# matthewygf/GPUSchedule

Hardware: NVIDIA H100
Metric: simulated events/sec (100k-job trace, 4x32x8 cluster) (higher is better)
Workload: dtype int32/int64 (+f64 durations)

## Files before the change

### gpuschedule_b200/csrc/gs_common.cuh

```cuda
#pragma once

#ifndef GS_TICK_MINBLOCKS
#define GS_TICK_MINBLOCKS 28
#endif
#ifndef GS_POLICY_MINBLOCKS
#define GS_POLICY_MINBLOCKS 20
#endif
#define FULL 0xffffffffu


struct __align__(32) JobIn {
  int arrive;
  int gpus;
  int gpc;
  int ps;
  long long memb;
  double dur;
};

struct PJob {
  int last_check, total_exec, exec, pending, last_pending, start, resume;
  unsigned char status, q_id, pad0, pad1;
};
enum { PST_NONE = 0, PST_PENDING = 1, PST_RUNNING = 2, PST_END = 3 };

struct SimDev {
  int M, G, K;
  int netcost, n, wheel_mask, policy, pad0;
  long long cap_bytes;
  long long fit_limit;
  double bandwidth, latency;
  const JobIn *jobs;
  const double *model_mb, *iters;
  gs_job_rec *rec;
  int *jstart;
  double *dur2;
  struct JobState2 *jst2;
  int *stack, *fin, *wheel_head;
  long long *wheel_mem;
  void *spans;
  gs_tick_row *rows;
  gs_evrow *evrows;
  gs_qrow *qrows;
  gs_nodeev *nodeev;
  unsigned long long *nbusy;
  int *nk;
  long long span_cap, rows_cap, qrows_cap;
  struct PJob *pj;
  int *runnable, *queues, *endj, *tmpl, *cidle, *ckfree;
  int *stalej;
  const double *git_data, *git_index;
  const double *git_direct;
  long long git_direct_n;
  double queue_limit[GS_MAX_QUEUES];
  double gittins_delta, next_gittins_unit;
  int num_queue, git_n, rn, en, end_time, next_job_jump, stale_n, qn[GS_MAX_QUEUES];
  int comm_rank, comm_n;
  int comm_min_runnable, comm_pad;
  long long comm_cap;
  double *comm_rk_in;
  unsigned long long *comm_flags;
  double *comm_peer_rk[GS_MAX_RANKS];
  unsigned long long *comm_peer_flags[GS_MAX_RANKS];
  unsigned long long comm_epoch;
  long long comm_wait_cycles;
  int delta, p, top, running, finished, ever, busy_gpus, done, status, need_init;
  int blocked;
  int nev, nq;
  int nne;
  long long mem_busy, sum_arr, span_used, events, evals, started, ticks, row_first;
};

#define EVER_BIT 0x80000000u
```

### gpuschedule_b200/csrc/gs_tick2.cuh

```cuda
#pragma once

#define SCACHE 4

struct __align__(16) JobState2 {
  int next;
  int where;
  unsigned long long mask0;
};

__device__ __forceinline__ unsigned lds32(unsigned a) { unsigned v; asm volatile("ld.shared.u32 %0, [%1];" : "=r"(v) : "r"(a)); return v; }
__device__ __forceinline__ void sts32(unsigned a, unsigned v) { asm volatile("st.shared.u32 [%0], %1;" :: "r"(a), "r"(v)); }
__device__ __forceinline__ unsigned long long lds64(unsigned a) { unsigned long long v; asm volatile("ld.shared.u64 %0, [%1];" : "=l"(v) : "r"(a)); return v; }
__device__ __forceinline__ void sts64(unsigned a, unsigned long long v) { asm volatile("st.shared.u64 [%0], %1;" :: "r"(a), "l"(v)); }
__device__ __forceinline__ int2 ldsv2(unsigned a) { int2 v; asm volatile("ld.shared.v2.s32 {%0, %1}, [%2];" : "=r"(v.x), "=r"(v.y) : "r"(a)); return v; }
__device__ __forceinline__ void stsv2(unsigned a, int2 v) { asm volatile("st.shared.v2.s32 [%0], {%1, %2};" :: "r"(a), "r"(v.x), "r"(v.y)); }

template <bool G64> struct MaskOps;
template <> struct MaskOps<true> {
  typedef unsigned long long T;
  typedef gs_span Span;
  static __device__ __forceinline__ Span make_span(int node, int ntasks, bool first, T mask) {
    Span sp; sp.node = node; sp.ntasks = ntasks | (first ? (int)0x80000000 : 0); sp.devmask = mask; return sp;
  }
  static __device__ __forceinline__ void st_span(Span *p, const Span &v) { __stcs(reinterpret_cast<int4 *>(p), *reinterpret_cast<const int4 *>(&v)); }
  static __device__ __forceinline__ int span_node(const Span &v) { return v.node; }
  static __device__ __forceinline__ int span_ntasks(const Span &v) { return v.ntasks & 0x7fffffff; }
  static __device__ __forceinline__ T span_mask(const Span &v) { return v.devmask; }
  static __device__ __forceinline__ T ld(unsigned a) { return lds64(a); }
  static __device__ __forceinline__ void st(unsigned a, T v) { sts64(a, v); }
  static __device__ __forceinline__ int popc(T v) { return __popcll(v); }
};
template <> struct MaskOps<false> {
  typedef unsigned T;
  typedef gs_cspan Span;
  static __device__ __forceinline__ Span make_span(int node, int ntasks, bool first, T mask) {
    Span sp; sp.where = (unsigned)node | ((unsigned)(ntasks - 1) << 20) | (first ? 0x80000000u : 0u); sp.devmask = mask; return sp;
  }
  static __device__ __forceinline__ void st_span(Span *p, const Span &v) { __stcs(reinterpret_cast<int2 *>(p), *reinterpret_cast<const int2 *>(&v)); }
  static __device__ __forceinline__ int span_node(const Span &v) { return (int)(v.where & 0xfffffu); }
  static __device__ __forceinline__ int span_ntasks(const Span &v) { return (int)((v.where >> 20) & 0x3fu) + 1; }
  static __device__ __forceinline__ T span_mask(const Span &v) { return v.devmask; }
// ... 14 lines not shown
}

__device__ __forceinline__ int meta_cap(unsigned mt, int gpc) {
  const int idle = (int)(mt & 0xffu), kfree = (int)(mt >> 16);
  return min(gpc == 1 ? idle : idle / gpc, kfree);
}

__device__ __forceinline__ int need_of(double dur) {
  const double cl = ceil(dur);
  return cl < 1.0 ? 1 : (cl > 1.0e9 ? 0x7fffffff : (int)cl);
}

#define GS_INF 0x7fffffff

template <bool NET, bool G64>
__global__ void __launch_bounds__(32, GS_TICK_MINBLOCKS) gs_tick2_kernel(SimDev *sims, int nsims, long long max_ticks, int smem_stride) {
  extern __shared__ __align__(16) unsigned char smem_raw[];
  typedef MaskOps<G64> MO;
  typedef typename MO::T MaskT;
  unsigned lane_u;
  asm volatile("mov.u32 %0, %%laneid;" : "=r"(lane_u));
  const int lane = (int)lane_u;
  const int sim = blockIdx.x;
  if (sim >= nsims) return;
  SimDev &S = sims[sim];
  if (S.done || S.status != 0 || S.policy != GS_SCHED_FIFO || (S.netcost != 0) != NET || (S.G > 32) != G64) return;

  const int M = S.M, G = S.G, n = S.n;
  unsigned sb_busy = (unsigned)__cvta_generic_to_shared(smem_raw);
  asm volatile("" : "+r"(sb_busy));
  unsigned sb_kk = sb_busy + 8u * (unsigned)M;
  asm volatile("" : "+r"(sb_kk));
  const unsigned sb_stk = sb_kk + 4u * (unsigned)(M + (M & 1));
#define BUSY_A(nd_) (sb_busy + 8u * (unsigned)(nd_))
#define KK_A(nd_) (sb_kk + 4u * (unsigned)(nd_))
#define STK_A(i_) (sb_stk + 8u * (unsigned)((i_) & (SCACHE - 1)))

  const JobIn *__restrict__ jobs = S.jobs;
  int *jstart = S.jstart;
  JobState2 *jst = S.jst2;
  int2 *stack = reinterpret_cast<int2 *>(S.stack);
  int *fin = S.fin, *whead = S.wheel_head;
  long long *wmem = S.wheel_mem;
  typedef typename MO::Span SpanT;
  SpanT *spans = reinterpret_cast<SpanT *>(S.spans);
  int2 *rowA = reinterpret_cast<int2 *>(S.evrows), *rowB = reinterpret_cast<int2 *>(S.qrows);
  int2 *nodeev = reinterpret_cast<int2 *>(S.nodeev);
  __builtin_assume(__isGlobal(jobs)); __builtin_assume(__isGlobal(jstart)); __builtin_assume(__isGlobal(jst));
  __builtin_assume(__isGlobal(stack)); __builtin_assume(__isGlobal(fin)); __builtin_assume(__isGlobal(whead));
  __builtin_assume(__isGlobal(wmem)); __builtin_assume(__isGlobal(spans)); __builtin_assume(__isGlobal(rowA));
  __builtin_assume(__isGlobal(rowB)); __builtin_assume(__isGlobal(nodeev));
  const int wmask = S.wheel_mask;
  const long long cap_bytes = S.cap_bytes, fit_limit = S.fit_limit;
  const int span_cap = (int)(S.span_cap > 0x7fffffffLL ? 0x7fffffffLL : S.span_cap);
  MaskT gmask = (G >= (int)(8 * sizeof(MaskT))) ? ~(MaskT)0 : (((MaskT)1 << G) - (MaskT)1);
  if constexpr (G64) asm volatile("" : "+l"(gmask));
  else asm volatile("" : "+r"(gmask));

  int delta = S.delta, p = S.p, top = S.top, running = S.running, finished = S.finished;
  int ever = S.ever, busy_gpus = S.busy_gpus, status = 0, blocked = S.blocked;
  int span_used = (int)S.span_used;
  long long mem_busy = S.mem_busy, sum_arr = S.sum_arr, evals = S.evals;
  const int delta0 = delta;
  const int capA = (int)(S.rows_cap > 0x7fffffffLL ? 0x7fffffffLL : S.rows_cap);
  const int capB = (int)(S.qrows_cap > 0x7fffffffLL ? 0x7fffffffLL : S.qrows_cap);
  int na = 0, nb = 0, nne = 0;
  int ever_rec = -1;
  long long budget_ll = max_ticks > 0 ? max_ticks : 0x7fffffffLL;
  if (budget_ll > 0x7fffffffLL - delta - 2) budget_ll = 0x7fffffffLL - delta - 2;
  const int t_end = delta + (int)(budget_ll > 0 ? budget_ll : 0);

  if (S.need_init) {
    const int K = S.K;
    for (int i = lane; i < M; i += 32) { sts64(BUSY_A(i), 0ull); sts32(KK_A(i), (unsigned)G | ((unsigned)K << 16)); }
    for (int i = lane; i <= wmask; i += 32) { whead[i] = -1; wmem[i] = 0; }
  } else {
    const int K = S.K;
    for (int i = lane; i < M; i += 32) {
      const unsigned long long bz = S.nbusy[i];
      const unsigned kv = (unsigned)S.nk[i];
      sts64(BUSY_A(i), bz);
      sts32(KK_A(i), (unsigned)(G - __popcll(bz)) | ((kv & EVER_BIT) ? 0x100u : 0u) | ((unsigned)(K - (int)(kv & ~EVER_BIT)) << 16));
    }
  }
  int scount = top;
  for (int i = max(scount - SCACHE, 0) + lane; i < scount; i += 32) stsv2(STK_A(i), stack[i]);
  int cache_lo = max(scount - SCACHE, 0);
  int bottom_arr = (top > 0) ? stack[0].y : 0;
  __syncwarp();

  int wbase = p & ~31;
  int warr = GS_INF, wpk = 1 | (1 << 24), wneed = 1, wps = 0;
  long long wmemc = 0;
  double wdur = 0.0;
#define LOAD_WINDOW()                                                                         \
  do {                                                                                        \
    warr = GS_INF;                                                                            \
    if (wbase + lane < n) {                                                                   \
      JobIn r_;                                                                               \
      {                                                                                       \
        const int4 *src_ = reinterpret_cast<const int4 *>(&jobs[wbase + lane]);               \
        const int4 v0_ = __ldcs(src_), v1_ = __ldcs(src_ + 1);             \
        r_.arrive = v0_.x; r_.gpus = v0_.y; r_.gpc = v0_.z; r_.ps = v0_.w;                     \
        r_.memb = (long long)(((unsigned long long)(unsigned)v1_.y << 32) | (unsigned)v1_.x); \
        r_.dur = __hiloint2double(v1_.w, v1_.z);                                              \
      }                                                                                       \
      warr = r_.arrive; wpk = r_.gpus | (r_.gpc << 24);                                       \
      wneed = need_of(r_.dur); if (!(r_.memb < fit_limit)) wneed = -wneed;                    \
      wmemc = (long long)r_.gpus * (r_.memb < cap_bytes ? r_.memb : cap_bytes);               \
      if (NET) { wdur = r_.dur; wps = r_.ps; }                                                \
    }                                                                                         \
  } while (0)
  LOAD_WINDOW();
  int next_arr = GS_INF;
  if (p < n) next_arr = __shfl_sync(FULL, warr, p - wbase);

  bool hvalid = false;
  int hjob = -1, harr = 0, hpk = 1 | (1 << 24), hneed = 1, hps = 0;
  long long hmemc = 0;
  double hdur = 0.0;
#define HEAD_FROM_WINDOW(src_)                                                                \
  do {                                                                                        \
    hpk = __shfl_sync(FULL, wpk, (src_)); hneed = __shfl_sync(FULL, wneed, (src_));           \
    hmemc = __shfl_sync(FULL, wmemc, (src_));                                                 \
    if (NET) { hdur = __longlong_as_double(__shfl_sync(FULL, __double_as_longlong(wdur), (src_))); hps = __shfl_sync(FULL, wps, (src_)); } \
  } while (0)

  int next_fin = GS_INF, nf_head = -1;
  JobState2 nf_js; nf_js.next = -1; nf_js.where = 0; nf_js.mask0 = 0ull;
  if (running > 0) {
    int base = delta + 1;
    while (true) {
      const int ph = whead[(base + lane) & wmask];
      const unsigned b = __ballot_sync(FULL, ph >= 0);
      if (b) { const int pos = __ffs(b) - 1; next_fin = base + pos; nf_head = __shfl_sync(FULL, ph, pos); break; }
      base += 32;
    }
    nf_js = jst[nf_head];
  }

  bool done = (n == 0);
  bool force = true;

  while (!done && status == 0) {
    if (na >= capA || nb >= capB) break;
    if (!force && (top == 0 || blocked)) {
      const int t_next = min(next_arr, next_fin - 1);
      if (t_next > delta) {
        const int t_to = min(t_next, t_end);
        if (blocked) evals += (long long)(t_to - delta) * M;
        delta = t_to;
      }
    }
    if (delta >= t_end) break;
    bool changed = force;
    force = false;
    if (next_arr <= delta) {
      int cnt = 0, q = p;
      while (true) {
        const int idx = wbase + lane;
        const unsigned b = __ballot_sync(FULL, idx >= q && warr <= delta);
        const int c = __popc(b);
        if (c > 0 && cnt == 0) {
          if (hvalid) {
            const int2 e = make_int2(hjob, harr);
            stack[scount] = e; stsv2(STK_A(scount), e);
            scount += 1;
          }
          HEAD_FROM_WINDOW(p - wbase);
        }
        cnt += c; q += c;
// ... 12 lines not shown
        if (scount - cache_lo > SCACHE) cache_lo = scount - SCACHE;
        if (top == 0) bottom_arr = delta;
        hjob = p; harr = delta; hvalid = true;
        top += cnt; p += cnt;
        sum_arr += (long long)cnt * delta;
        blocked = 0; changed = true;
        __syncwarp();
      }
      next_arr = GS_INF;
      if (p < n) next_arr = __shfl_sync(FULL, warr, p - wbase);
    }
    if (top > 0 && blocked) evals += M;
    if (top > 0 && !blocked) {
      if (!hvalid) {
        int2 e;
        if (scount - 1 >= cache_lo) e = ldsv2(STK_A(scount - 1));
        else e = stack[scount - 1];
        scount -= 1;
        if (cache_lo > scount) cache_lo = scount;
        hjob = e.x; harr = e.y; hvalid = true;
        if (hjob >= wbase && hjob < wbase + 32) {
          HEAD_FROM_WINDOW(hjob - wbase);
        } else {
          const JobIn jr = jobs[hjob];
          hpk = jr.gpus | (jr.gpc << 24);
          hneed = need_of(jr.dur); if (!(jr.memb < fit_limit)) hneed = -hneed;
          hmemc = (long long)jr.gpus * (jr.memb < cap_bytes ? jr.memb : cap_bytes);
          if (NET) { hdur = jr.dur; hps = jr.ps; }
        }
      }
      const int hg = hpk & 0xffffff, hgpc = (int)((unsigned)hpk >> 24);
      const int htasks = hgpc == 1 ? hg : hg / hgpc;
      const bool placeable = hneed > 0;
      int pre_bk = 0, pre_head = -1;
      long long pre_wm = 0;
      if (!NET && placeable) {
        pre_bk = (delta + min(hneed, wmask)) & wmask;
        pre_head = whead[pre_bk];
        pre_wm = wmem[pre_bk];
      }
      bool ok = false;
      int nspans = 0, where = 0;
      const int span_first = span_used;
      unsigned long long mask0 = 0;
      if (hg <= G) {
        int found = -1;
        for (int base = 0; base < M; base += 32) {
          const int nd = base + lane;
          bool fit = false;
          if (nd < M) {
            const unsigned mt = lds32(KK_A(nd));
            fit = (int)(mt & 0xffu) >= hg && (int)(mt >> 16) >= htasks;
          }
          if (!placeable) {
            if (fit) sts32(KK_A(nd), lds32(KK_A(nd)) - ((unsigned)htasks << 16));
            continue;
          }
          const unsigned b = __ballot_sync(FULL, fit);
          if (b) { found = base + __ffs(b) - 1; break; }
        }
        if (found >= 0 && span_used + 1 > span_cap) { status = GS_ERR_CAPACITY; found = -1; }
        if (found >= 0) {
          ok = true; nspans = 1;
          const MaskT bz = MO::ld(BUSY_A(found));
          const MaskT take = take_lowest<MaskT>(~bz & gmask, hg);
          const unsigned kv = lds32(KK_A(found));
          MO::st(BUSY_A(found), bz | take);
          sts32(KK_A(found), (kv - (unsigned)hg - ((unsigned)htasks << 16)) | 0x100u);
          MO::st_span(&spans[span_first], MO::make_span(found, htasks, true, take));
          mask0 = take;
          where = found | ((htasks - 1) << 20);
          ever += (kv & 0x100u) ? 0 : 1;
          evals += found + 1;
        } else {
          evals += M;
        }
      } else {
// ... 11 lines not shown
            if (nd < M) { const unsigned mt = lds32(KK_A(nd)); if (meta_cap(mt, hgpc) > 0) sts32(KK_A(nd), mt - (1u << 16)); }
          }
        }
        if (last_base >= 0 && (long long)span_used + min(htasks, M) > (long long)span_cap) { status = GS_ERR_CAPACITY; last_base = -1; }
        if (last_base >= 0) {
          ok = true;
          int rem = htasks, last_node = 0;
          for (int base = 0; base <= last_base; base += 32) {
            const int nd = base + lane;
            const unsigned kv = (nd < M) ? lds32(KK_A(nd)) : 0u;
            const int c = meta_cap(kv, hgpc);
            int incl = c;
            #pragma unroll
            for (int o = 1; o < 32; o <<= 1) { const int v = __shfl_up_sync(FULL, incl, o); if (lane >= o) incl += v; }
            const int take = min(c, max(rem - (incl - c), 0));
            const unsigned tb = __ballot_sync(FULL, take > 0);
            bool fresh = false;
            if (take > 0) {
              const MaskT bz = MO::ld(BUSY_A(nd));
              const MaskT tk = take_lowest<MaskT>(~bz & gmask, take * hgpc);
              MO::st(BUSY_A(nd), bz | tk);
              sts32(KK_A(nd), (kv - (unsigned)(take * hgpc) - ((unsigned)take << 16)) | 0x100u);
              fresh = !(kv & 0x100u);
              const int slot = nspans + __popc(tb & ((1u << lane) - 1u));
              MO::st_span(&spans[span_first + slot], MO::make_span(nd, take, slot == 0, tk));
            }
            ever += __popc(__ballot_sync(FULL, fresh));
            if (tb) last_node = base + 31 - __clz(tb);
            nspans += __popc(tb);
            const int tot = __shfl_sync(FULL, incl, 31);
            rem -= min(rem, tot);
          }
          where = (int)0x80000000 | span_first;
          mask0 = (unsigned long long)(unsigned)nspans | ((unsigned long long)(unsigned)hg << 32);
          evals += last_node + 1;
          __syncwarp();
        } else {
          evals += M;
          __syncwarp();
        }
      }
      if (ok) {
        const int j = hjob;
        int need = hneed;
        if (NET) {
          double dur2 = hdur;
          if (hps > 1) {
            const double mps = __ddiv_rn(S.model_mb[j], S.bandwidth);
            const double nis = __dmul_rn((double)nspans, S.latency);
            const double rt = __dmul_rn(S.iters[j], 2.0);
            dur2 = __dadd_rn(hdur, __dmul_rn(__dadd_rn(mps, nis), rt));
          }
          const double eff = dur2 > hdur ? dur2 : hdur;
          need = need_of(eff);
          S.dur2[j] = dur2;
        }
        if (need > wmask) { status = GS_ERR_ARG; need = wmask; }
        const int endt = delta + need;
        const int bk = endt & wmask;
        span_used += nspans;
        JobState2 js; js.where = where; js.mask0 = mask0; js.next = -1;
        if (endt < next_fin) { next_fin = endt; nf_head = j; nf_js = js; }
        else if (endt == next_fin) { js.next = nf_head; nf_head = j; nf_js = js; }
        else js.next = NET ? whead[bk] : pre_head;
        const long long wm = NET ? wmem[bk] : pre_wm;
        whead[bk] = j;
        wmem[bk] = wm + hmemc;
        *reinterpret_cast<int4 *>(&jst[j]) = *reinterpret_cast<const int4 *>(&js);
        __stcs(&jstart[j], delta);
        top -= 1;
        sum_arr -= harr;
        running += 1;
        busy_gpus += hg;
        mem_busy += hmemc;
        hvalid = false; changed = true;
      } else if (placeable) {
        blocked = 1;
      }
    }
    const int now = delta + 1;
    if (next_fin == now) {
      const int sl = now & wmask;
      int ph = whead[(now + 1 + lane) & wmask];
      const long long wm = wmem[sl];
      int h = nf_head;
      JobState2 js = nf_js;
      const int f0 = finished;
      int c = 0;
      while (true) {
        if (js.where >= 0) {
          const int nd = js.where & 0xfffff, nt = ((js.where >> 20) & 63) + 1;
          const int gp = __popcll(js.mask0);
          const MaskT bz = MO::ld(BUSY_A(nd));
          const unsigned kv = lds32(KK_A(nd));
          MO::st(BUSY_A(nd), bz & ~(MaskT)js.mask0);
          sts32(KK_A(nd), kv + (unsigned)gp + ((unsigned)nt << 16));
          busy_gpus -= gp;
        } else {
          const int first = js.where & 0x7fffffff, scnt = (int)(unsigned)(js.mask0 & 0xffffffffull);
          for (int i = lane; i < scnt; i += 32) {
            const SpanT sp = spans[first + i];
            const int snd = MO::span_node(sp);
            const MaskT smk = MO::span_mask(sp);
            MO::st(BUSY_A(snd), MO::ld(BUSY_A(snd)) & ~smk);
            sts32(KK_A(snd), lds32(KK_A(snd)) + (unsigned)MO::popc(smk) + ((unsigned)MO::span_ntasks(sp) << 16));
          }
          busy_gpus -= (int)(unsigned)(js.mask0 >> 32);
          __syncwarp();
        }
        fin[f0 + c] = h;
        c += 1;
        h = js.next;
        if (h < 0) break;
        js = jst[h];
      }
      finished += c; running -= c;
      mem_busy -= wm;
      whead[sl] = -1; wmem[sl] = 0;
      if (c >= 2) {
        for (int i = lane; i < (c >> 1); i += 32) { const int a = fin[f0 + i], b2 = fin[f0 + c - 1 - i]; fin[f0 + i] = b2; fin[f0 + c - 1 - i] = a; }
        __syncwarp();
      }
      next_fin = GS_INF; nf_head = -1;
      if (running > 0) {
        int base = now + 1;
        while (true) {
          const unsigned b = __ballot_sync(FULL, ph >= 0);
          if (b) { const int pos = __ffs(b) - 1; next_fin = base + pos; nf_head = __shfl_sync(FULL, ph, pos); break; }
          base += 32;
          ph = whead[(base + lane) & wmask];
        }
        nf_js = jst[nf_head];
      }
      blocked = 0; changed = true;
    }
    if (changed) {
      if (top > 0) {
        const int ilo = top - 1 - ((top - 1) >> 1), ihi = top - 1 - (top >> 1);
        int a_lo, a_hi;
        if (hvalid && ilo == top - 1) a_lo = harr;
        else a_lo = ilo >= cache_lo ? ldsv2(STK_A(ilo)).y : stack[ilo].y;
        if (hvalid && ihi == top - 1) a_hi = harr;
        else a_hi = ihi >= cache_lo ? ldsv2(STK_A(ihi)).y : stack[ihi].y;
        {
          int2 *qb = rowB + 3 * nb;
          __stcs(qb, make_int2(now, bottom_arr));
          __stcs(qb + 1, make_int2(a_lo, a_hi));
          __stcs(qb + 2, make_int2((int)(sum_arr & 0xffffffffLL), (int)(sum_arr >> 32)));
        }
        nb += 1;
      }
      if (ever != ever_rec) { __stcs(&nodeev[nne], make_int2(now, ever)); nne += 1; ever_rec = ever; }
      {
        int2 *ab = rowA + 3 * na;
        __stcs(ab, make_int2(now, top));
        __stcs(ab + 1, make_int2(finished, busy_gpus | (running << 16)));
        __stcs(ab + 2, make_int2((int)(mem_busy & 0xffffffffLL), (int)(mem_busy >> 32)));
      }
      na += 1;
    }
    delta = now;
    done = (n - p) + running == 0;
  }
#undef LOAD_WINDOW
#undef HEAD_FROM_WINDOW

  __syncwarp();
  if (hvalid) { if (lane == 0) stack[scount] = make_int2(hjob, harr); scount += 1; }
  __syncwarp();
  for (int i = lane; i < scount; i += 32) jstart[stack[i].x] = -1;
  {
    const int K = S.K;
    for (int i = lane; i < M; i += 32) {
      const unsigned mt = lds32(KK_A(i));
      S.nbusy[i] = (unsigned long long)MO::ld(BUSY_A(i));
      S.nk[i] = (int)((unsigned)(K - (int)(mt >> 16)) | ((mt & 0x100u) ? EVER_BIT : 0u));
    }
  }
  if (lane == 0) {
    S.delta = delta; S.p = p; S.top = top; S.running = running; S.finished = finished;
    S.ever = ever; S.busy_gpus = busy_gpus; S.mem_busy = mem_busy; S.sum_arr = sum_arr;
    S.span_used = span_used; S.started = (long long)finished + running;
    S.events = (long long)p + finished + running + finished; S.evals = evals;
    S.ticks = delta; S.row_first = delta0; S.nev = na; S.nq = nb; S.nne = nne; S.blocked = blocked;
    S.done = done ? 1 : 0; S.status = status; S.need_init = 0;
  }
#undef BUSY_A
#undef KK_A
#undef STK_A
}

__global__ void gs_expand_rows_kernel(const SimDev *sims, int sim, int M, int G, gs_tick_row *__restrict__ out) {
  const SimDev &S = sims[sim];
  const int na = S.nev;
  const int k = blockIdx.x * blockDim.x + threadIdx.x;
  if (k >= na) return;
  const gs_evrow a = S.evrows[k];
  const int t_first = a.now;
  const int t_last = (k + 1 < na) ? S.evrows[k + 1].now - 1 : (int)S.ticks;
  const int queued = a.queued, busy_gpus = a.busy_gpus, running = a.running;
  int nodes = 0;
  {
    int lo = 0, hi = S.nne - 1;
    while (lo < hi) { const int mid = (lo + hi + 1) >> 1; if (S.nodeev[mid].now <= t_first) lo = mid; else hi = mid - 1; }
    if (S.nne > 0) nodes = S.nodeev[lo].busy_nodes;
  }
  long long sum_arr = 0; int bottom = 0, a_lo = 0, a_hi = 0;
  if (queued > 0) {
    int lo = 0, hi = S.nq - 1;
    while (lo < hi) { const int mid = (lo + hi) >> 1; if (S.qrows[mid].now < t_first) lo = mid + 1; else hi = mid; }
    const gs_qrow b = S.qrows[lo];
    sum_arr = b.arrive_sum; bottom = b.oldest_arrive; a_lo = b.med_lo_arrive; a_hi = b.med_hi_arrive;
  }
  const long long row0 = S.row_first;
  for (int v = t_first; v <= t_last; ++v) {
    int4 *dst = reinterpret_cast<int4 *>(&out[(long long)v - 1 - row0]);
    const long long ps = queued > 0 ? (long long)queued * v - sum_arr : 0;
    dst[0] = make_int4(v, M - nodes, nodes, busy_gpus);
    dst[1] = make_int4(M * G - busy_gpus, running, queued, a.finished);
    dst[2] = make_int4((int)(a.mem_busy_bytes & 0xffffffffLL), (int)(a.mem_busy_bytes >> 32), (int)(ps & 0xffffffffLL), (int)(ps >> 32));
    dst[3] = queued > 0 ? make_int4(v - bottom, v - a_lo, v - a_hi, 0) : make_int4(0, 0, 0, 0);
  }
// ... 20 lines not shown
```

### gpuschedule_b200/csrc/gsched.cu

```cuda
#include <cuda_runtime.h>
#include <stdint.h>
#include <stdio.h>
#include <stdlib.h>
#include <string.h>

#include <algorithm>
#include <string>
#include <vector>

#include "gsched.h"

#include "gs_common.cuh"
#include "gs_tick2.cuh"
#include "gs_policy.cuh"
#include "gs_aux.cuh"
#include "gs_switch.cuh"
#include "gs_summary.cuh"
#include "gs_boot.cuh"


struct SimLayout {
  size_t o_ev = 0, o_q = 0, o_ne = 0, o_rec2 = 0, o_dur2 = 0, o_fin = 0, o_spans = 0, out_bytes = 0;
  size_t o_rec = 0, o_rows = 0, o_jst = 0, o_stack = 0, o_wh = 0, o_wm = 0, o_nb = 0, o_nk = 0;
  size_t o_pj = 0, o_run = 0, o_qs = 0, o_end = 0, o_tmp = 0, o_ci = 0, o_ck = 0, o_stale = 0;
  size_t total = 0;
  int64_t rows_cap = 0, qrows_cap = 0;
  int W = 256;
};

struct SimHost {
  gs_cluster cl;
  gs_policy pol;
  bool configured = false, loaded = false, prepared = false;
  int64_t n = 0;
  void *trace_slab = nullptr;
  void *state_slab = nullptr;
  void *git_dev = nullptr;
  long long git_direct_n = 0;
  size_t trace_bytes = 0, state_bytes = 0;
  int64_t span_cap = 0, rows_cap = 0, qrows_cap = 0, last_arrive = 0;
  int max_need = 1;
  unsigned char *state_ptr = nullptr;
  bool trace_in_arena = false;
  int64_t sum_rows = 0;
  bool sum_fresh = true;
  bool tl_fresh = true;
  bool tl_done = false;
  bool jd_done = false;
  bool sd_done = false;
  bool occ_fresh = true;
  bool occ_done = false;
  SimDev dev;
  SimLayout layout;
};

struct gs_engine {
  int device = 0, nsims = 0;
  cudaStream_t stream = nullptr;
  cudaEvent_t e0 = nullptr, e1 = nullptr;
  cudaEvent_t e_wait = nullptr;
// ... 307 lines not shown
  if (h->span_budget > 0) {
    const int64_t lim = (int64_t)(h->span_budget * (double)n) + 4096;
    if (span_cap > lim) span_cap = lim;
  }
  s.n = n; s.span_cap = span_cap > 0 ? span_cap : 1;
  s.max_need = (int)max_need + 2;
  s.last_arrive = n > 0 ? ji[n - 1].arrive : 0;
  s.loaded = true;
  s.trace_in_arena = false;
  s.prepared = false;
  h->dirty = true;
  return GS_OK;
}

extern "C" int gs_load_trace(gs_handle h, int sim, int64_t n, const int32_t *arrive_tick, const int32_t *gpus,
                             const int32_t *gpu_per_task, const double *duration, const int64_t *mem_bytes,
                             const double *model_mb, const double *iterations, const int32_t *ps_count) {
  return load_common(h, sim, n, nullptr, arrive_tick, gpus, gpu_per_task, duration, mem_bytes, model_mb, iterations, ps_count);
}

extern "C" int gs_load_trace_packed(gs_handle h, int sim, int64_t n, const gs_jobin *jobs, const double *model_mb,
                                    const double *iterations) {
  static_assert(sizeof(gs_jobin) == sizeof(JobIn), "gs_jobin layout");
  if (n > 0 && !jobs) return fail(h, GS_ERR_ARG, "gs_load_trace_packed: NULL records");
  return load_common(h, sim, n, reinterpret_cast<const JobIn *>(jobs), nullptr, nullptr, nullptr, nullptr, nullptr,
                     model_mb, iterations, nullptr);
}

static SimLayout layout_sim(gs_handle h, const SimHost &s, int64_t rows_cap) {
  SimLayout L;
  const gs_cluster &c = s.cl;
  const int M = c.num_switch * c.num_node_p_switch;
  const size_t N = (size_t)(s.n > 0 ? s.n : 1);
  int W = 256; while (W < s.max_need + 1) W <<= 1;
  L.W = W;
  if (rows_cap <= 0) rows_cap = s.last_arrive + 2ll * s.max_need + 4096;
  L.rows_cap = rows_cap;
  L.qrows_cap = h->qrows_cap > 0 ? h->qrows_cap : rows_cap;
  const bool evd = s.pol.schedule != GS_SCHED_FIFO;
  const bool net = c.enable_network_costs != 0;
  size_t total = 0;
  auto take = [&](size_t bytes) { const size_t o = total; total = align_up(total + bytes); return o; };
  if (evd) {
    L.o_fin = take(4 * N);
    L.o_rec = take(sizeof(gs_job_rec) * N);
    L.o_rows = take(sizeof(gs_tick_row) * (size_t)rows_cap);
    L.out_bytes = total;
    const size_t nql = (size_t)(s.pol.num_queue > 2 ? s.pol.num_queue : 2);
    L.o_pj = take(sizeof(PJob) * N); L.o_run = take(4 * N); L.o_qs = take(4 * N * nql); L.o_end = take(4 * N);
    L.o_tmp = take(4 * N); L.o_ci = take(4 * (size_t)M); L.o_ck = take(4 * (size_t)M); L.o_stale = take(4 * N);
  } else {
    L.o_ev = take(sizeof(gs_evrow) * (size_t)rows_cap);
    L.o_q = take(sizeof(gs_qrow) * (size_t)L.qrows_cap);
    L.o_ne = take(sizeof(gs_nodeev) * (size_t)(M + 2));
    L.o_rec2 = take(4 * N);
    if (net) L.o_dur2 = take(8 * N);
    L.o_fin = take(4 * N);
    L.o_spans = take((c.num_gpu_p_node > 32 ? sizeof(gs_span) : sizeof(gs_cspan)) * (size_t)s.span_cap);
    L.out_bytes = total;
    L.o_jst = take(sizeof(JobState2) * N);
    L.o_stack = take(8 * (N + 1));
    L.o_wh = take(4 * (size_t)W); L.o_wm = take(8 * (size_t)W);
    L.o_nb = take(8 * (size_t)M); L.o_nk = take(4 * (size_t)M);
  }
  L.total = total;
  return L;
}

static int bind_sim(gs_handle h, SimHost &s, const SimLayout &L, unsigned char *d) {
  const gs_cluster &c = s.cl;
  const int M = c.num_switch * c.num_node_p_switch;
  const int W = L.W;
  const int64_t rows_cap = L.rows_cap, qrows_cap = L.qrows_cap;
  const bool evd = s.pol.schedule != GS_SCHED_FIFO;
  const bool net = c.enable_network_costs != 0;
  const size_t o_fin = L.o_fin, o_rec = L.o_rec, o_rows = L.o_rows, o_rec2 = L.o_rec2, o_dur2 = L.o_dur2, o_jst = L.o_jst, o_stack = L.o_stack;
  const size_t o_wh = L.o_wh, o_wm = L.o_wm, o_spans = L.o_spans, o_ev = L.o_ev, o_q = L.o_q, o_nb = L.o_nb, o_nk = L.o_nk;
  const size_t o_pj = L.o_pj, o_run = L.o_run, o_qs = L.o_qs, o_end = L.o_end, o_tmp = L.o_tmp, o_ci = L.o_ci, o_ck = L.o_ck, o_stale = L.o_stale;
  s.layout = L;
  s.state_ptr = d;
  SimDev &D = s.dev;
  D.M = M; D.G = c.num_gpu_p_node;
  int kc = c.num_cpu_p_node / c.cpu_per_task, km = c.mem_p_node / c.mem_per_task;
  D.K = kc < km ? kc : km;
  D.netcost = net ? 1 : 0;
  D.n = (int)s.n; D.wheel_mask = W - 1; D.policy = s.pol.schedule;
  D.cap_bytes = (long long)c.gpu_mem_cap_mib << 20;
  D.fit_limit = D.cap_bytes - ((long long)500 << 20);
  D.bandwidth = c.bandwidth; D.latency = c.internode_latency;
  D.fin = (int *)(d + o_fin);
  D.rec = nullptr; D.rows = nullptr; D.jstart = nullptr; D.dur2 = nullptr; D.jst2 = nullptr; D.stack = nullptr;
  D.wheel_head = nullptr; D.wheel_mem = nullptr; D.spans = nullptr; D.evrows = nullptr; D.qrows = nullptr; D.nodeev = nullptr; D.nbusy = nullptr; D.nk = nullptr;
  if (evd) {
    D.rec = (gs_job_rec *)(d + o_rec); D.rows = (gs_tick_row *)(d + o_rows);
  } else {
    D.jstart = (int *)(d + o_rec2); D.dur2 = net ? (double *)(d + o_dur2) : nullptr;
    D.jst2 = (JobState2 *)(d + o_jst); D.stack = (int *)(d + o_stack);
    D.wheel_head = (int *)(d + o_wh); D.wheel_mem = (long long *)(d + o_wm);
    D.spans = (void *)(d + o_spans); D.evrows = (gs_evrow *)(d + o_ev); D.qrows = (gs_qrow *)(d + o_q); D.nodeev = (gs_nodeev *)(d + L.o_ne);
    D.nbusy = (unsigned long long *)(d + o_nb); D.nk = (int *)(d + o_nk);
  }
  D.span_cap = s.span_cap; D.rows_cap = rows_cap; D.qrows_cap = qrows_cap;
  s.rows_cap = rows_cap; s.qrows_cap = qrows_cap;
  if (evd) {
    D.pj = (PJob *)(d + o_pj); D.runnable = (int *)(d + o_run); D.queues = (int *)(d + o_qs);
    D.endj = (int *)(d + o_end); D.tmpl = (int *)(d + o_tmp); D.cidle = (int *)(d + o_ci); D.ckfree = (int *)(d + o_ck);
    D.stalej = (int *)(d + o_stale); D.stale_n = 0;
    D.num_queue = s.pol.num_queue > 0 ? s.pol.num_queue : 1;
    for (int q = 0; q < GS_MAX_QUEUES; ++q) { D.queue_limit[q] = s.pol.queue_limit[q]; D.qn[q] = 0; }
    D.gittins_delta = s.pol.gittins_delta; D.next_gittins_unit = s.pol.gittins_delta;
    D.git_n = s.pol.schedule == GS_SCHED_GITTINS ? s.pol.gittins_n : 0;
    D.git_data = (const double *)s.git_dev;
    D.git_index = s.git_dev ? (const double *)((unsigned char *)s.git_dev + 8 * (size_t)s.pol.gittins_n) : nullptr;
    D.git_direct_n = (s.git_dev && D.git_n > 0) ? s.git_direct_n : 0;
    D.git_direct = D.git_direct_n > 0 ? (const double *)((unsigned char *)s.git_dev + 16 * (size_t)s.pol.gittins_n) : nullptr;
    D.rn = 0; D.en = 0; D.end_time = 0x7fffffff; D.next_job_jump = 0x7fffffff;
  }
  D.comm_n = 0; D.comm_rank = 0; D.comm_cap = 0; D.comm_rk_in = nullptr; D.comm_flags = nullptr; D.comm_epoch = 0; D.comm_wait_cycles = 0;
  if (h->comm_n > 1 && s.pol.schedule == GS_SCHED_GITTINS) {
    if ((int64_t)s.n > h->comm_cap) return fail(h, GS_ERR_ARG, "gs_run: the trace has more jobs than gs_comm_prepare sized the exchange buffer for");
    D.comm_epoch = h->comm_epoch; h->comm_epoch0 = h->comm_epoch;
    D.comm_n = h->comm_n; D.comm_rank = h->comm_rank; D.comm_cap = h->comm_cap; D.comm_min_runnable = h->comm_min_runnable;
    D.comm_flags = (unsigned long long *)h->comm_buf;
    D.comm_rk_in = (double *)((unsigned char *)h->comm_buf + 256);
    for (int q = 0; q < h->comm_n; ++q) {
      D.comm_peer_flags[q] = (unsigned long long *)h->comm_peer[q];
      D.comm_peer_rk[q] = (double *)((unsigned char *)h->comm_peer[q] + 256);
    }
  }
  D.delta = D.p = D.top = D.running = D.finished = D.ever = D.busy_gpus = D.done = D.status = 0;
  D.blocked = D.nev = D.nq = D.nne = 0;
// ... 53 lines not shown
    if (s.pol.schedule == GS_SCHED_FIFO) fifo_kind[(s.cl.enable_network_costs ? 2 : 0) + (s.cl.num_gpu_p_node > 32 ? 1 : 0)] = true;
    else { any_evd = true; evd_init |= s.dev.need_init != 0; }
  }
  if (h->dirty) {
    for (int i = 0; i < h->nsims; ++i) h->h_back[(size_t)i] = h->sims[(size_t)i].dev;
    CU(cudaMemcpyAsync(h->d_sims, h->h_back.data(), sizeof(SimDev) * (size_t)h->nsims, cudaMemcpyHostToDevice, h->stream));
    CU(cudaStreamSynchronize(h->stream));
    h->dirty = false;
  }
  CU(cudaEventRecord(h->e0, h->stream));
  if (any_evd) {
    if (evd_init) {
      gs_init_kernel<<<dim3(16, (unsigned)h->nsims), 256, 0, h->stream>>>(h->d_sims, h->nsims);
      CU(cudaGetLastError());
      h->launches += 1;
    }
    const int thread_map = h->engine_mode == 2 ? 1 : 0;
    if (thread_map) {
      gs_policy_kernel<<<(unsigned)((h->nsims + 31) / 32), 32, 0, h->stream>>>(h->d_sims, h->nsims, (long long)max_ticks, 1);
      CU(cudaGetLastError());
      h->launches += 1;
    } else {
      gs_dlas_warp_kernel<<<(unsigned)h->nsims, 32, 0, h->stream>>>(h->d_sims, h->nsims, (long long)max_ticks);
      CU(cudaGetLastError());
      const size_t pol_smem = 8 * (size_t)maxM;
      if (pol_smem > 48 * 1024)
        CU(cudaFuncSetAttribute(gs_sortpol_warp_kernel, cudaFuncAttributeMaxDynamicSharedMemorySize, (int)pol_smem));
      gs_sortpol_warp_kernel<<<(unsigned)h->nsims, 32, pol_smem, h->stream>>>(h->d_sims, h->nsims, (long long)max_ticks);
      CU(cudaGetLastError());
      h->launches += 2;
    }
  }
  if (fifo_kind[0] || fifo_kind[1] || fifo_kind[2] || fifo_kind[3]) {
    const int stride = (int)align_up((size_t)maxM * 12 + 8 + SCACHE * 8, 16);
    if (stride > 200 * 1024) return fail(h, GS_ERR_ARG, "gs_run: node table does not fit shared memory (M too large)");
#define GS_LAUNCH_TICK2(NET_, G64_)                                                                                              \
    do {                                                                                                                         \
      if (stride > 48 * 1024) CU(cudaFuncSetAttribute(gs_tick2_kernel<NET_, G64_>, cudaFuncAttributeMaxDynamicSharedMemorySize, stride)); \
      gs_tick2_kernel<NET_, G64_><<<(unsigned)h->nsims, 32, (size_t)stride, h->stream>>>(h->d_sims, h->nsims, (long long)max_ticks, stride); \
      CU(cudaGetLastError());                                                                                                    \
      h->launches += 1;                                                                                                          \
    } while (0)
    if (fifo_kind[0]) GS_LAUNCH_TICK2(false, false);
    if (fifo_kind[1]) GS_LAUNCH_TICK2(false, true);
    if (fifo_kind[2]) GS_LAUNCH_TICK2(true, false);
    if (fifo_kind[3]) GS_LAUNCH_TICK2(true, true);
#undef GS_LAUNCH_TICK2
  }
  CU(cudaEventRecord(h->e1, h->stream));
  CU(cudaMemcpyAsync(h->h_back.data(), h->d_sims, sizeof(SimDev) * (size_t)h->nsims, cudaMemcpyDeviceToHost, h->stream));
  CU(wait_stream(h));
  float ms = 0; cudaEventElapsedTime(&ms, h->e0, h->e1);
  h->kernel_ms += ms;
  if (h->comm_n > 1 && h->h_back[0].comm_n > 1) h->comm_epoch = h->h_back[0].comm_epoch;
  int worst = 0;
  for (int i = 0; i < h->nsims; ++i) {
    h->h_back[(size_t)i].need_init = 0;
    h->sims[(size_t)i].dev = h->h_back[(size_t)i];
    if (h->h_back[(size_t)i].status != 0 && worst == 0) worst = h->h_back[(size_t)i].status;
  }
  if (worst != 0) return fail(h, worst, "gs_run: a replica stopped with an in-kernel error (see gs_stats.status)");
  return GS_OK;
}

extern "C" int gs_stats(gs_handle h, int sim, gs_run_stats *out) {
  if (!h || !out) return GS_ERR_ARG;
  if (sim < 0 || sim >= h->nsims) return fail(h, GS_ERR_ARG, "gs_stats: sim index out of range");
// ... 1163 lines not shown
```

Before: 5.124 billion.

## Replace timing-wheel finish lists with a shared-memory running-job slot table

Removes the global timing wheel (bucket heads, bucket memory and per-job linked list) from the FIFO tick kernel. Running jobs are now kept in a RunSlot table: the first 32 slots live in shared memory, one per lane, and the rest overflow to global memory. Finishing jobs are found with warp ballots over the slots, and the next finish time comes from a warp min-reduction. This avoids scattered global bucket walks, at the cost of linear scans over the global overflow slots on every finish tick whenever more than 32 jobs are running, plus an extra start-time tie-break search when several jobs finish in the same tick.

Measured after the change: 5.399 billion, median of 6. +5.4%, better.

```diff
diff --git a/gpuschedule_b200/csrc/gs_common.cuh b/gpuschedule_b200/csrc/gs_common.cuh
--- a/gpuschedule_b200/csrc/gs_common.cuh
+++ b/gpuschedule_b200/csrc/gs_common.cuh
@@ -26,7 +26,7 @@
 
 struct SimDev {
   int M, G, K;
-  int netcost, n, wheel_mask, policy, pad0;
+  int netcost, n, policy, pad0;
   long long cap_bytes;
   long long fit_limit;
   double bandwidth, latency;
@@ -35,9 +35,8 @@
   gs_job_rec *rec;
   int *jstart;
   double *dur2;
-  struct JobState2 *jst2;
-  int *stack, *fin, *wheel_head;
-  long long *wheel_mem;
+  struct RunSlot *runtab;
+  int *stack, *fin;
   void *spans;
   gs_tick_row *rows;
   gs_evrow *evrows;
@@ -72,3 +71,14 @@
 };
 
 #define EVER_BIT 0x80000000u
+
+struct __align__(16) RunSlot {
+  int fin;
+  int start;
+  int job;
+  int where;
+  unsigned long long mask;
+  long long mem;
+};
+#define GS_RUN_SMEM 32
+static_assert(GS_RUN_SMEM == 32, "gs_tick2_kernel gives every lane one shared slot and tracks them in a 32-bit mask");
diff --git a/gpuschedule_b200/csrc/gs_tick2.cuh b/gpuschedule_b200/csrc/gs_tick2.cuh
--- a/gpuschedule_b200/csrc/gs_tick2.cuh
+++ b/gpuschedule_b200/csrc/gs_tick2.cuh
@@ -1,12 +1,6 @@
 #pragma once
 
 #define SCACHE 4
-
-struct __align__(16) JobState2 {
-  int next;
-  int where;
-  unsigned long long mask0;
-};
 
 __device__ __forceinline__ unsigned lds32(unsigned a) { unsigned v; asm volatile("ld.shared.u32 %0, [%1];" : "=r"(v) : "r"(a)); return v; }
 __device__ __forceinline__ void sts32(unsigned a, unsigned v) { asm volatile("st.shared.u32 [%0], %1;" :: "r"(a), "r"(v)); }
@@ -87,25 +81,45 @@
   unsigned sb_kk = sb_busy + 8u * (unsigned)M;
   asm volatile("" : "+r"(sb_kk));
   const unsigned sb_stk = sb_kk + 4u * (unsigned)(M + (M & 1));
+  const unsigned sb_rt = sb_stk + 8u * SCACHE;
 #define BUSY_A(nd_) (sb_busy + 8u * (unsigned)(nd_))
 #define KK_A(nd_) (sb_kk + 4u * (unsigned)(nd_))
 #define STK_A(i_) (sb_stk + 8u * (unsigned)((i_) & (SCACHE - 1)))
+#define RT_FS(i_) (sb_rt + 8u * (unsigned)(i_))
+#define RT_JW(i_) (sb_rt + 8u * GS_RUN_SMEM + 8u * (unsigned)(i_))
+#define RT_MEM(i_) (sb_rt + 16u * GS_RUN_SMEM + 8u * (unsigned)(i_))
+#define RT_MSK(i_) (sb_rt + 24u * GS_RUN_SMEM + (unsigned)sizeof(MaskT) * (unsigned)(i_))
+  auto rt_get = [&](int i) {
+    RunSlot v;
+    if (i < GS_RUN_SMEM) {
+      const int2 fs = ldsv2(RT_FS(i)), jw = ldsv2(RT_JW(i));
+      v.fin = fs.x; v.start = fs.y; v.job = jw.x; v.where = jw.y;
+      v.mem = (long long)lds64(RT_MEM(i)); v.mask = MO::ld(RT_MSK(i));
+    } else {
+      v = S.runtab[i];
+    }
+    return v;
+  };
+  auto rt_put = [&](int i, const RunSlot &v) {
+    if (i < GS_RUN_SMEM) {
+      stsv2(RT_FS(i), make_int2(v.fin, v.start)); stsv2(RT_JW(i), make_int2(v.job, v.where));
+      sts64(RT_MEM(i), (unsigned long long)v.mem); MO::st(RT_MSK(i), (MaskT)v.mask);
+    } else {
+      S.runtab[i] = v;
+    }
+  };
 
   const JobIn *__restrict__ jobs = S.jobs;
   int *jstart = S.jstart;
-  JobState2 *jst = S.jst2;
   int2 *stack = reinterpret_cast<int2 *>(S.stack);
-  int *fin = S.fin, *whead = S.wheel_head;
-  long long *wmem = S.wheel_mem;
+  int *fin = S.fin;
   typedef typename MO::Span SpanT;
   SpanT *spans = reinterpret_cast<SpanT *>(S.spans);
   int2 *rowA = reinterpret_cast<int2 *>(S.evrows), *rowB = reinterpret_cast<int2 *>(S.qrows);
   int2 *nodeev = reinterpret_cast<int2 *>(S.nodeev);
-  __builtin_assume(__isGlobal(jobs)); __builtin_assume(__isGlobal(jstart)); __builtin_assume(__isGlobal(jst));
-  __builtin_assume(__isGlobal(stack)); __builtin_assume(__isGlobal(fin)); __builtin_assume(__isGlobal(whead));
-  __builtin_assume(__isGlobal(wmem)); __builtin_assume(__isGlobal(spans)); __builtin_assume(__isGlobal(rowA));
+  __builtin_assume(__isGlobal(jobs)); __builtin_assume(__isGlobal(jstart));
+  __builtin_assume(__isGlobal(stack)); __builtin_assume(__isGlobal(fin)); __builtin_assume(__isGlobal(spans)); __builtin_assume(__isGlobal(rowA));
   __builtin_assume(__isGlobal(rowB)); __builtin_assume(__isGlobal(nodeev));
-  const int wmask = S.wheel_mask;
   const long long cap_bytes = S.cap_bytes, fit_limit = S.fit_limit;
   const int span_cap = (int)(S.span_cap > 0x7fffffffLL ? 0x7fffffffLL : S.span_cap);
   MaskT gmask = (G >= (int)(8 * sizeof(MaskT))) ? ~(MaskT)0 : (((MaskT)1 << G) - (MaskT)1);
@@ -128,7 +142,6 @@
   if (S.need_init) {
     const int K = S.K;
     for (int i = lane; i < M; i += 32) { sts64(BUSY_A(i), 0ull); sts32(KK_A(i), (unsigned)G | ((unsigned)K << 16)); }
-    for (int i = lane; i <= wmask; i += 32) { whead[i] = -1; wmem[i] = 0; }
   } else {
     const int K = S.K;
     for (int i = lane; i < M; i += 32) {
@@ -181,17 +194,16 @@
     if (NET) { hdur = __longlong_as_double(__shfl_sync(FULL, __double_as_longlong(wdur), (src_))); hps = __shfl_sync(FULL, wps, (src_)); } \
   } while (0)
 
-  int next_fin = GS_INF, nf_head = -1;
-  JobState2 nf_js; nf_js.next = -1; nf_js.where = 0; nf_js.mask0 = 0ull;
-  if (running > 0) {
-    int base = delta + 1;
-    while (true) {
-      const int ph = whead[(base + lane) & wmask];
-      const unsigned b = __ballot_sync(FULL, ph >= 0);
-      if (b) { const int pos = __ffs(b) - 1; next_fin = base + pos; nf_head = __shfl_sync(FULL, ph, pos); break; }
-      base += 32;
-    }
-    nf_js = jst[nf_head];
+  int next_fin;
+  unsigned occ;
+  {
+    int nf = GS_INF;
+    if (S.need_init) sts32(RT_FS(lane), (unsigned)GS_INF);
+    else { const RunSlot v = S.runtab[lane]; rt_put(lane, v); nf = v.fin; }
+    occ = __ballot_sync(FULL, nf != GS_INF);
+    for (int i = GS_RUN_SMEM + lane; i < GS_RUN_SMEM + running - __popc(occ); i += 32) nf = min(nf, S.runtab[i].fin);
+    next_fin = __reduce_min_sync(FULL, nf);
+    __syncwarp();
   }
 
   bool done = (n == 0);
@@ -270,17 +282,10 @@
       const int hg = hpk & 0xffffff, hgpc = (int)((unsigned)hpk >> 24);
       const int htasks = hgpc == 1 ? hg : hg / hgpc;
       const bool placeable = hneed > 0;
-      int pre_bk = 0, pre_head = -1;
-      long long pre_wm = 0;
-      if (!NET && placeable) {
-        pre_bk = (delta + min(hneed, wmask)) & wmask;
-        pre_head = whead[pre_bk];
-        pre_wm = wmem[pre_bk];
-      }
       bool ok = false;
       int nspans = 0, where = 0;
       const int span_first = span_used;
-      unsigned long long mask0 = 0;
+      MaskT mask0 = 0;
       if (hg <= G) {
         int found = -1;
         for (int base = 0; base < M; base += 32) {
@@ -358,7 +363,7 @@
             rem -= min(rem, tot);
           }
           where = (int)0x80000000 | span_first;
-          mask0 = (unsigned long long)(unsigned)nspans | ((unsigned long long)(unsigned)hg << 32);
+          mask0 = (MaskT)nspans;
           evals += last_node + 1;
           __syncwarp();
         } else {
@@ -381,18 +386,19 @@
           need = need_of(eff);
           S.dur2[j] = dur2;
         }
-        if (need > wmask) { status = GS_ERR_ARG; need = wmask; }
         const int endt = delta + need;
-        const int bk = endt & wmask;
         span_used += nspans;
-        JobState2 js; js.where = where; js.mask0 = mask0; js.next = -1;
-        if (endt < next_fin) { next_fin = endt; nf_head = j; nf_js = js; }
-        else if (endt == next_fin) { js.next = nf_head; nf_head = j; nf_js = js; }
-        else js.next = NET ? whead[bk] : pre_head;
-        const long long wm = NET ? wmem[bk] : pre_wm;
-        whead[bk] = j;
-        wmem[bk] = wm + hmemc;
-        *reinterpret_cast<int4 *>(&jst[j]) = *reinterpret_cast<const int4 *>(&js);
+        {
+          RunSlot v; v.fin = endt; v.start = delta; v.job = j; v.where = where; v.mask = mask0; v.mem = hmemc;
+          if (occ != FULL) {
+            const int k = __ffs(~occ) - 1;
+            occ |= 1u << k;
+            rt_put(k, v);
+          } else {
+            rt_put(running + GS_RUN_SMEM - 32, v);
+          }
+        }
+        next_fin = min(next_fin, endt);
         __stcs(&jstart[j], delta);
         top -= 1;
         sum_arr -= harr;
@@ -406,57 +412,73 @@
     }
     const int now = delta + 1;
     if (next_fin == now) {
-      const int sl = now & wmask;
-      int ph = whead[(now + 1 + lane) & wmask];
-      const long long wm = wmem[sl];
-      int h = nf_head;
-      JobState2 js = nf_js;
-      const int f0 = finished;
-      int c = 0;
       while (true) {
-        if (js.where >= 0) {
-          const int nd = js.where & 0xfffff, nt = ((js.where >> 20) & 63) + 1;
-          const int gp = __popcll(js.mask0);
+        const int f0 = (int)lds32(RT_FS(lane));
+        const unsigned b0 = __ballot_sync(FULL, f0 == now);
+        int nf = f0 == now ? GS_INF : f0;
+        int c = __popc(b0);
+        int i = __ffs(b0) - 1;
+        const int tend = GS_RUN_SMEM + running - __popc(occ);
+        if (tend > GS_RUN_SMEM) {
+          #pragma unroll 1
+          for (int base = GS_RUN_SMEM; base < tend; base += 32) {
+            const int k = base + lane;
+            const int f = k < tend ? S.runtab[k].fin : GS_INF;
+            const unsigned b = __ballot_sync(FULL, f == now);
+            if (b && c == 0) i = base + __ffs(b) - 1;
+            c += __popc(b);
+            if (f != now) nf = min(nf, f);
+          }
+        }
+        if (c == 0) { next_fin = __reduce_min_sync(FULL, nf); break; }
+        if (c > 1) {
+          const int2 fs = ldsv2(RT_FS(lane));
+          int key = fs.x == now ? fs.y : GS_INF, kslot = lane;
+          #pragma unroll 1
+          for (int k = GS_RUN_SMEM + lane; k < tend; k += 32) {
+            const int2 ft = make_int2(S.runtab[k].fin, S.runtab[k].start);
+            if (ft.x == now && ft.y < key) { key = ft.y; kslot = k; }
+          }
+          const int kmin = __reduce_min_sync(FULL, key);
+          i = __shfl_sync(FULL, kslot, __ffs(__ballot_sync(FULL, key == kmin)) - 1);
+        }
+        RunSlot v;
+        if (i < GS_RUN_SMEM) {
+          const int2 jw = ldsv2(RT_JW(i));
+          v.job = jw.x; v.where = jw.y; v.mem = (long long)lds64(RT_MEM(i)); v.mask = MO::ld(RT_MSK(i));
+          sts32(RT_FS(i), (unsigned)GS_INF);
+          occ &= ~(1u << i);
+        } else {
+          v = S.runtab[i];
+          if (i < tend - 1) S.runtab[i] = S.runtab[tend - 1];
+        }
+        if (v.where >= 0) {
+          const int nd = v.where & 0xfffff, nt = ((v.where >> 20) & 63) + 1;
+          const MaskT mk = (MaskT)v.mask;
+          const int gp = MO::popc(mk);
           const MaskT bz = MO::ld(BUSY_A(nd));
           const unsigned kv = lds32(KK_A(nd));
-          MO::st(BUSY_A(nd), bz & ~(MaskT)js.mask0);
+          MO::st(BUSY_A(nd), bz & ~mk);
           sts32(KK_A(nd), kv + (unsigned)gp + ((unsigned)nt << 16));
           busy_gpus -= gp;
         } else {
-          const int first = js.where & 0x7fffffff, scnt = (int)(unsigned)(js.mask0 & 0xffffffffull);
-          for (int i = lane; i < scnt; i += 32) {
-            const SpanT sp = spans[first + i];
+          const int first = v.where & 0x7fffffff, scnt = (int)v.mask;
+          int gp = 0;
+          for (int k = lane; k < scnt; k += 32) {
+            const SpanT sp = spans[first + k];
             const int snd = MO::span_node(sp);
             const MaskT smk = MO::span_mask(sp);
             MO::st(BUSY_A(snd), MO::ld(BUSY_A(snd)) & ~smk);
             sts32(KK_A(snd), lds32(KK_A(snd)) + (unsigned)MO::popc(smk) + ((unsigned)MO::span_ntasks(sp) << 16));
-          }
-          busy_gpus -= (int)(unsigned)(js.mask0 >> 32);
+            gp += MO::popc(smk);
+          }
+          busy_gpus -= __reduce_add_sync(FULL, gp);
           __syncwarp();
         }
-        fin[f0 + c] = h;
-        c += 1;
-        h = js.next;
-        if (h < 0) break;
-        js = jst[h];
-      }
-      finished += c; running -= c;
-      mem_busy -= wm;
-      whead[sl] = -1; wmem[sl] = 0;
-      if (c >= 2) {
-        for (int i = lane; i < (c >> 1); i += 32) { const int a = fin[f0 + i], b2 = fin[f0 + c - 1 - i]; fin[f0 + i] = b2; fin[f0 + c - 1 - i] = a; }
-        __syncwarp();
-      }
-      next_fin = GS_INF; nf_head = -1;
-      if (running > 0) {
-        int base = now + 1;
-        while (true) {
-          const unsigned b = __ballot_sync(FULL, ph >= 0);
-          if (b) { const int pos = __ffs(b) - 1; next_fin = base + pos; nf_head = __shfl_sync(FULL, ph, pos); break; }
-          base += 32;
-          ph = whead[(base + lane) & wmask];
-        }
-        nf_js = jst[nf_head];
+        fin[finished] = v.job;
+        finished += 1; running -= 1;
+        mem_busy -= v.mem;
+        if (c == 1) { next_fin = __reduce_min_sync(FULL, nf); break; }
       }
       blocked = 0; changed = true;
     }
@@ -495,6 +517,7 @@
   if (hvalid) { if (lane == 0) stack[scount] = make_int2(hjob, harr); scount += 1; }
   __syncwarp();
   for (int i = lane; i < scount; i += 32) jstart[stack[i].x] = -1;
+  S.runtab[lane] = rt_get(lane);
   {
     const int K = S.K;
     for (int i = lane; i < M; i += 32) {
@@ -514,6 +537,10 @@
 #undef BUSY_A
 #undef KK_A
 #undef STK_A
+#undef RT_FS
+#undef RT_JW
+#undef RT_MEM
+#undef RT_MSK
 }
 
 __global__ void gs_expand_rows_kernel(const SimDev *sims, int sim, int M, int G, gs_tick_row *__restrict__ out) {
diff --git a/gpuschedule_b200/csrc/gsched.cu b/gpuschedule_b200/csrc/gsched.cu
--- a/gpuschedule_b200/csrc/gsched.cu
+++ b/gpuschedule_b200/csrc/gsched.cu
@@ -21,11 +21,10 @@
 
 struct SimLayout {
   size_t o_ev = 0, o_q = 0, o_ne = 0, o_rec2 = 0, o_dur2 = 0, o_fin = 0, o_spans = 0, out_bytes = 0;
-  size_t o_rec = 0, o_rows = 0, o_jst = 0, o_stack = 0, o_wh = 0, o_wm = 0, o_nb = 0, o_nk = 0;
+  size_t o_rec = 0, o_rows = 0, o_rt = 0, o_stack = 0, o_nb = 0, o_nk = 0;
   size_t o_pj = 0, o_run = 0, o_qs = 0, o_end = 0, o_tmp = 0, o_ci = 0, o_ck = 0, o_stale = 0;
   size_t total = 0;
   int64_t rows_cap = 0, qrows_cap = 0;
-  int W = 256;
 };
 
 struct SimHost {
@@ -399,8 +398,6 @@
   const gs_cluster &c = s.cl;
   const int M = c.num_switch * c.num_node_p_switch;
   const size_t N = (size_t)(s.n > 0 ? s.n : 1);
-  int W = 256; while (W < s.max_need + 1) W <<= 1;
-  L.W = W;
   if (rows_cap <= 0) rows_cap = s.last_arrive + 2ll * s.max_need + 4096;
   L.rows_cap = rows_cap;
   L.qrows_cap = h->qrows_cap > 0 ? h->qrows_cap : rows_cap;
@@ -425,9 +422,10 @@
     L.o_fin = take(4 * N);
     L.o_spans = take((c.num_gpu_p_node > 32 ? sizeof(gs_span) : sizeof(gs_cspan)) * (size_t)s.span_cap);
     L.out_bytes = total;
-    L.o_jst = take(sizeof(JobState2) * N);
+    const int kc = c.num_cpu_p_node / c.cpu_per_task, km = c.mem_p_node / c.mem_per_task;
+    const int64_t slots = (int64_t)M * (kc < km ? kc : km);
+    L.o_rt = take(sizeof(RunSlot) * (size_t)(GS_RUN_SMEM + std::max<int64_t>(std::min<int64_t>((int64_t)N, slots), 0)));
     L.o_stack = take(8 * (N + 1));
-    L.o_wh = take(4 * (size_t)W); L.o_wm = take(8 * (size_t)W);
     L.o_nb = take(8 * (size_t)M); L.o_nk = take(4 * (size_t)M);
   }
   L.total = total;
@@ -437,12 +435,11 @@
 static int bind_sim(gs_handle h, SimHost &s, const SimLayout &L, unsigned char *d) {
   const gs_cluster &c = s.cl;
   const int M = c.num_switch * c.num_node_p_switch;
-  const int W = L.W;
   const int64_t rows_cap = L.rows_cap, qrows_cap = L.qrows_cap;
   const bool evd = s.pol.schedule != GS_SCHED_FIFO;
   const bool net = c.enable_network_costs != 0;
-  const size_t o_fin = L.o_fin, o_rec = L.o_rec, o_rows = L.o_rows, o_rec2 = L.o_rec2, o_dur2 = L.o_dur2, o_jst = L.o_jst, o_stack = L.o_stack;
-  const size_t o_wh = L.o_wh, o_wm = L.o_wm, o_spans = L.o_spans, o_ev = L.o_ev, o_q = L.o_q, o_nb = L.o_nb, o_nk = L.o_nk;
+  const size_t o_fin = L.o_fin, o_rec = L.o_rec, o_rows = L.o_rows, o_rec2 = L.o_rec2, o_dur2 = L.o_dur2, o_rt = L.o_rt, o_stack = L.o_stack;
+  const size_t o_spans = L.o_spans, o_ev = L.o_ev, o_q = L.o_q, o_nb = L.o_nb, o_nk = L.o_nk;
   const size_t o_pj = L.o_pj, o_run = L.o_run, o_qs = L.o_qs, o_end = L.o_end, o_tmp = L.o_tmp, o_ci = L.o_ci, o_ck = L.o_ck, o_stale = L.o_stale;
   s.layout = L;
   s.state_ptr = d;
@@ -451,19 +448,18 @@
   int kc = c.num_cpu_p_node / c.cpu_per_task, km = c.mem_p_node / c.mem_per_task;
   D.K = kc < km ? kc : km;
   D.netcost = net ? 1 : 0;
-  D.n = (int)s.n; D.wheel_mask = W - 1; D.policy = s.pol.schedule;
+  D.n = (int)s.n; D.policy = s.pol.schedule;
   D.cap_bytes = (long long)c.gpu_mem_cap_mib << 20;
   D.fit_limit = D.cap_bytes - ((long long)500 << 20);
   D.bandwidth = c.bandwidth; D.latency = c.internode_latency;
   D.fin = (int *)(d + o_fin);
-  D.rec = nullptr; D.rows = nullptr; D.jstart = nullptr; D.dur2 = nullptr; D.jst2 = nullptr; D.stack = nullptr;
-  D.wheel_head = nullptr; D.wheel_mem = nullptr; D.spans = nullptr; D.evrows = nullptr; D.qrows = nullptr; D.nodeev = nullptr; D.nbusy = nullptr; D.nk = nullptr;
+  D.rec = nullptr; D.rows = nullptr; D.jstart = nullptr; D.dur2 = nullptr; D.runtab = nullptr; D.stack = nullptr;
+  D.spans = nullptr; D.evrows = nullptr; D.qrows = nullptr; D.nodeev = nullptr; D.nbusy = nullptr; D.nk = nullptr;
   if (evd) {
     D.rec = (gs_job_rec *)(d + o_rec); D.rows = (gs_tick_row *)(d + o_rows);
   } else {
     D.jstart = (int *)(d + o_rec2); D.dur2 = net ? (double *)(d + o_dur2) : nullptr;
-    D.jst2 = (JobState2 *)(d + o_jst); D.stack = (int *)(d + o_stack);
-    D.wheel_head = (int *)(d + o_wh); D.wheel_mem = (long long *)(d + o_wm);
+    D.runtab = (RunSlot *)(d + o_rt); D.stack = (int *)(d + o_stack);
     D.spans = (void *)(d + o_spans); D.evrows = (gs_evrow *)(d + o_ev); D.qrows = (gs_qrow *)(d + o_q); D.nodeev = (gs_nodeev *)(d + L.o_ne);
     D.nbusy = (unsigned long long *)(d + o_nb); D.nk = (int *)(d + o_nk);
   }
@@ -583,7 +579,7 @@
     }
   }
   if (fifo_kind[0] || fifo_kind[1] || fifo_kind[2] || fifo_kind[3]) {
-    const int stride = (int)align_up((size_t)maxM * 12 + 8 + SCACHE * 8, 16);
+    const int stride = (int)align_up((size_t)maxM * 12 + 8 + SCACHE * 8 + GS_RUN_SMEM * (16 + 8 + 8), 16);
     if (stride > 200 * 1024) return fail(h, GS_ERR_ARG, "gs_run: node table does not fit shared memory (M too large)");
 #define GS_LAUNCH_TICK2(NET_, G64_)                                                                                              \
     do {                                                                                                                         \
```
